# PREDICT-EPFL/polympc

Hardware: AMD Instinct MI355X
Metric: box-ADMM QP subproblem solves/s (fused SQP hot path) (higher is better)
Workload: dtype f64

## Files before the change

polympc_amd/csrc/pmpc_launch.hpp:

```cpp
#pragma once
#include <hip/hip_runtime.h>
#include <cstdlib>
#include "../../include/polympc_amd.h"
#include "pmpc_ocp.hpp"
#include "pmpc_qp.hpp"
#include "pmpc_qp_reg.hpp"
#include "pmpc_qp_reg2.hpp"
#include "pmpc_qp_cond.hpp"
#include "pmpc_qp_big.hpp"
#include "pmpc_sqp.hpp"

extern "C" pmpc_status pmpc_internal_services(pmpc_context* ctx, int P, int S, double t0, double tf, size_t ws_bytes, const void** cheb,
                                               double** ws, void** stream, size_t* lds_limit, unsigned long long** phase_cycles, int* force_lds);
extern "C" int pmpc_internal_simd_count(pmpc_context* ctx);
extern "C" int pmpc_internal_sqp_slice(pmpc_context* ctx);
extern "C" int pmpc_internal_sqp_rr(pmpc_context* ctx);
extern "C" void pmpc_internal_set_route(pmpc_context* ctx, int route);
extern "C" int pmpc_internal_last_route(pmpc_context* ctx);
enum { PMPC_SW_NO_REDO_LAUNCH = 0, PMPC_SW_NO_CONDREG = 1, PMPC_SW_NO_SCHUR = 2, PMPC_SW_SCHUR_SMALL = 3, PMPC_SW_BIG_WG4_ON = 4, PMPC_SW_BIG_WG4_OFF = 5, PMPC_SW_NO_CONDREG_RUIZ = 6 };
extern "C" int pmpc_internal_switch(pmpc_context* ctx, int which);

namespace pmpc {
using ::pmpc_status;

// ... 6 lines not shown
}

template <int NN, int MM, int NNODES> constexpr int cond_qp_staging() {
    if constexpr (NN <= WAVE) return RegKkt<NN>::TRI;
    else {
        constexpr int a = RegKkt2<NN, PMPC_COND_NV>::TRI, b = CondDims<NN, MM>::TAB_OFF + CondDims<NN, MM>::template tab_doubles<NNODES>();
        return a > b ? a : b;
    }
}

template <int NN, int MM, int NNODES, int NX> constexpr int cond_qp_staging_ws() {
    constexpr int a = cond_qp_staging<NN, MM, NNODES>(), b = CondDims<NN, MM>::TAB_OFF + CondDims<NN, MM>::template tab_doubles_ws<NNODES, NX>();
    return a > b ? a : b;
}

template <class Model> __host__ __device__ inline size_t jview_doubles(int nnodes) {
    return (size_t)nnodes * (Model::NX + Model::NG) * OcpDims<Model>::JBS;
}

template <class Model> __host__ __device__ inline size_t big_scratch_doubles(int P, int S) {
    OcpDims<Model> dm(P, S);
    return ((SqpLds::doubles(dm.n, dm.m, dm.mi) + OcpLds<Model>::doubles(P, S) + QpLds::doubles_rest(dm.n, dm.m) + jview_doubles<Model>(dm.NN) + 8) + 1) & ~(size_t)1;
}

template <class Model, int NN = 0, int MM = 0, unsigned V = 0>
#ifndef PMPC_SQP_WAVES
#define PMPC_SQP_WAVES 2
#endif
#ifndef PMPC_BIG_WAVES
#define PMPC_BIG_WAVES 1
#endif
#ifndef PMPC_COND1_WAVES
#define PMPC_COND1_WAVES 1
#endif
__global__ __launch_bounds__((V & SQP_TEAM4) ? 256 : 64, ((NN > 0 && NN + MM <= 64) ? PMPC_SQP_WAVES : ((NN > 0 && (V & SQP_COND) && NN <= 64) ? PMPC_COND1_WAVES : (((V & SQP_HBM) && (V & SQP_TWO_WAVES)) ? 2 : ((V & SQP_HBM) ? PMPC_BIG_WAVES : 1))))) void sqp_kernel(Model model, const ChebData* __restrict__ cd, int B,
                                                 const double* __restrict__ x_guess, const double* __restrict__ lam_guess,
                                                 const double* __restrict__ d, const double* __restrict__ lbx,
                                                 const double* __restrict__ ubx, const double* __restrict__ lbg,
                                                 const double* __restrict__ ubg, pmpc_sqp_settings ss, pmpc_qp_settings qs,
                                                 double* __restrict__ Hws, double* __restrict__ Aws, double* __restrict__ x,
                                                 double* __restrict__ lam, pmpc_sqp_info* __restrict__ info, unsigned long long* __restrict__ phase_cycles,
                                                 double* __restrict__ Kws, int it_begin, int it_end, double* __restrict__ slice_state, unsigned lds_dyn_doubles) {
    static_assert(sqp_variant_ok<NN, V>(), "sqp_kernel: variant flags that no launcher route selects");
    constexpr bool PROF = (V & SQP_PROF) != 0, KHBM = (V & SQP_HBM) != 0, POL = (V & SQP_HOOKS) != 0, CND = (V & SQP_COND) != 0, WG4 = (V & SQP_TEAM4) != 0;
    extern __shared__ double smem[];
    const size_t lds_doubles_total = __builtin_amdgcn_groupstaticsize() / sizeof(double) + lds_dyn_doubles;
    const int b = blockIdx.x;
    if (b >= B) return;
    int flags0 = 0;
    if (it_begin == PMPC_REDO_MODE) { if (__builtin_amdgcn_readfirstlane(info[b].status) != PMPC_SQP_REDO) return; it_begin = 0; flags0 = PMPC_FLAG_ILLCOND; }
    if (it_begin != 0 && __builtin_amdgcn_readfirstlane(info[b].status) != PMPC_SQP_IN_PROGRESS) return;
    if (it_begin < 0) it_begin = __builtin_amdgcn_readfirstlane(info[b].iter);
    const int P = cd->P, S = cd->S;
    Ocp<Model> ocp(model, P, S, cd->t_scale);
    const int n = ocp.dm.n, m = ocp.dm.m, mi = ocp.dm.mi;
    QpLds qw; SqpLds v;
    double* p; double* stage0; const double* stage_end; double* big_mail = nullptr;
    if constexpr (NN == 0 && KHBM) {
        p = qw.carve_xy(smem, n, m);
        double* rhsL = p; p += n + m;
        qw.big_lds = p; p += BigKkt::LDS_DOUBLES;
        big_mail = p; p += BIG_MAIL_DOUBLES;
        ocp.Dlds = p; p += (size_t)(P + 1) * (P + 2);
        if constexpr (Model::NG == 0 && Model::NP == 0) { if (JViewRT<Model>::tab_worth_it(ocp.dm.NN)) { p += (p - smem) & 1; ocp.jtab = p; p += JViewRT<Model>::tab_doubles(ocp.dm.NN); } }
        double* Wb = Kws + (size_t)b * (BigKkt::doubles(n + m) + big_scratch_doubles<Model>(P, S));
        double* hq = Wb + BigKkt::doubles(n + m);
        hq = v.carve(hq, n, m, mi);
        stage0 = hq;
        hq = ocp.s.carve(hq, P, S);
        stage_end = hq;
        qw.carve_rest_split(hq, rhsL, n, m, Wb);
        hq += QpLds::doubles_rest(n, m);
        ocp.jblk = hq; ocp.gblk = ocp.jblk + (size_t)ocp.dm.NN * Model::NX * OcpDims<Model>::JBS; ocp.keep_blk = true;
    } else {
        p = (NN > 0) ? qw.carve_xy(smem, n, m) : qw.carve(smem, n, ss.qp_solver == 1 ? m + n : m);
        p = v.carve(p, n, m, mi);
        stage0 = p;
        p = ocp.s.carve(p, P, S);
        constexpr int QP_STAGING0 = []() constexpr {
            if constexpr (CND) return cond_qp_staging<NN, MM, NN / (Model::NX + Model::NU)>();
            else return reg_qp_staging<NN + MM>(); }();
        int QP_STAGING = QP_STAGING0;
        if constexpr (CND && POL) {
            if (ss.preconditioner == 1) QP_STAGING = cond_qp_staging_ws<NN, MM, NN / (Model::NX + Model::NU), Model::NX>();
        }
        if (NN > 0 && (size_t)(p - stage0) < (size_t)QP_STAGING + 2 + ocp.s.const_doubles(P, S)) p = stage0 + QP_STAGING + 2 + ocp.s.const_doubles(P, S);
        stage_end = p;
    }
    if constexpr (NN > 0 && (NN + MM > WAVE || CND)) {
        ocp.jblk = p; p += jview_doubles<Model>(ocp.dm.NN); ocp.gblk = ocp.jblk + (size_t)ocp.dm.NN * Model::NX * OcpDims<Model>::JBS; ocp.keep_blk = true;
    }
    double* dL = p; p += (Model::ND > 0 ? Model::ND : 1);
    const int ln = lane_id();
    ocp.d = dL;
    double* filt = nullptr;
    if constexpr (NN == 0 || POL) { filt = p; p += FILTER_LDS_DOUBLES; }
    if constexpr (WG4) {
        if (threadIdx.x >= WAVE) { big_helper_loop<Model>((BigMail<JViewRT<Model>>*)big_mail, (int)(threadIdx.x >> 6), ocp); return; }
    }
    for (int i = ln; i < Model::ND; i += WAVE) dL[i] = d[(size_t)b * Model::ND + i];
    if constexpr (NN == 0 || POL) {
        const bool carried = ss.line_search == 1 && ss.filter_state != nullptr;
        if (ln < PMPC_FILTER_STATE_DOUBLES) filt[ln] = carried ? ss.filter_state[(size_t)b * PMPC_FILTER_STATE_DOUBLES + ln] : 0.0;
    }
    double* eigw = nullptr;
    if constexpr (NN == 0 || POL) { if (ss.regularisation == 1) { eigw = p; p += 2 * (size_t)n * n; } }
    ocp.stage_constants(cd);
    if constexpr (NN == 0 && KHBM) {
        for (int i = ln; i < (P + 1) * (P + 2); i += WAVE) ocp.Dlds[i] = ocp.s.D[i];
        wsync();
        if constexpr (Model::NG == 0 && Model::NP == 0) { if (JViewRT<Model>::tab_worth_it(ocp.dm.NN)) JViewRT<Model>::build_tables(ocp.Dlds, P, ocp.dm.NN, ocp.jtab); }
    }
    double* sst = slice_state ? slice_state + (size_t)b * 2 * n : nullptr;
    constexpr bool BOUNDS_RULE = NN > 0 && (CND || NN + MM <= WAVE);
    bool loose = false;
    for (int i = ln; i < n; i += WAVE) {
        v.x[i] = (it_begin > 0) ? x[(size_t)b * n + i] : (x_guess ? x_guess[(size_t)b * n + i] : 0.0);
        const double lbi = lbx[(size_t)b * n + i], ubi = ubx[(size_t)b * n + i];
        v.lbx[i] = lbi; v.ubx[i] = ubi;
        if constexpr (BOUNDS_RULE) loose |= (i >= ocp.dm.VARX) && (lbi < -LOOSE_BOUNDS_THRESH) && (ubi > LOOSE_BOUNDS_THRESH);
        if (it_begin > 0) { v.lg[i] = sst[i]; v.step[i] = sst[n + i]; }
    }
    for (int i = ln; i < m + n; i += WAVE)
        v.lam[i] = (it_begin > 0) ? lam[(size_t)b * (m + n) + i] : (lam_guess ? lam_guess[(size_t)b * (m + n) + i] : 0.0);
    for (int i = ln; i < mi; i += WAVE) {
        v.lbg[i] = lbg ? lbg[(size_t)b * mi + i] : -INFINITY;
        v.ubg[i] = ubg ? ubg[(size_t)b * mi + i] : INFINITY;
    }
    wsync();
    if constexpr (BOUNDS_RULE) {
        if (it_begin == 0 && flags0 == 0 && __builtin_amdgcn_ballot_w64(loose) != 0) {
            for (int i = ln; i < n; i += WAVE) x[(size_t)b * n + i] = v.x[i];
            for (int i = ln; i < m + n; i += WAVE) lam[(size_t)b * (m + n) + i] = v.lam[i];
            if (ln == 0) { pmpc_sqp_info r; r.iter = 0; r.qp_solver_iter = 0; r.status = PMPC_SQP_REDO; r.flags = PMPC_FLAG_ILLCOND; r.primal_norm = 0.0; r.dual_norm = 0.0; r.max_violation = 0.0; r.cost = 0.0; info[b] = r; }
            return;
        }
    }
    double* K0 = Hws + (size_t)b * (size_t)(n + m) * n;
    (void)Aws;
    SqpDevice<Model, NN, MM, V> sqp(ocp, v, qw, K0, K0 + n, ss, qs);
    sqp.big_mail = big_mail;
    sqp.filt = filt;
    sqp.eig = eigw;
    sqp.trace = ss.iteration_trace ? ss.iteration_trace + (size_t)b * (size_t)ss.iteration_trace_capacity * PMPC_TRACE_DOUBLES : nullptr;
    sqp.tr = ocp.s.fval;
    if constexpr (NN + MM > 112) sqp.tr += (ocp.s.fval - smem) & 1;
    {
        const int G = WAVE / ocp.dm.NN;
        const size_t need = (size_t)G * (m + ocp.dm.NN + 3);
        const size_t have = (size_t)(stage_end - ocp.s.fval);
        sqp.lsbuf = ocp.s.fval;
        sqp.ls_side_by_side = (G >= 2 && need <= have);
        sqp.ls_wide = sqp.ls_side_by_side && need + (size_t)2 * G * n <= have;
    }
    pmpc_sqp_info si;
    sqp.qp_flags = flags0;
    if (it_begin > 0) { const pmpc_sqp_info prev = info[b]; sqp.qp_iter_total = prev.qp_solver_iter; sqp.qp_flags = prev.flags; sqp.cost_log = prev.cost; }
    sqp.solve(si, it_begin, it_end);
    if (si.status == PMPC_SQP_IN_PROGRESS && sst) for (int i = ln; i < n; i += WAVE) { sst[i] = v.lg[i]; sst[n + i] = v.step[i]; }
    for (int i = ln; i < n; i += WAVE) x[(size_t)b * n + i] = v.x[i];
    for (int i = ln; i < m + n; i += WAVE) lam[(size_t)b * (m + n) + i] = v.lam[i];
    if (ln == 0) info[b] = si;
    if constexpr (NN == 0 || POL) {
        if (ss.line_search == 1 && ss.filter_state != nullptr && si.status != PMPC_SQP_REDO && ln < PMPC_FILTER_STATE_DOUBLES) ss.filter_state[(size_t)b * PMPC_FILTER_STATE_DOUBLES + ln] = filt[ln];
    }
    if constexpr (PROF) { if (phase_cycles && ln == 0) for (int i = 0; i < 24; ++i) atomicAdd(&phase_cycles[i], (unsigned long long)sqp.cyc[i]); }
    if constexpr (WG4) {
        if (ln == 0) ((BigMail<JViewRT<Model>>*)big_mail)->op = BIG_OP_EXIT;
        __syncthreads();
    }
}
template <class Model, int PP, int SS> constexpr int schur_lds_doubles_ct() {
    using SD = SchurDims<Model, PP, SS>;
    return SD::LDS_DOUBLES + SD::NNODES * SD::DD  + (SD::NPAR ? 2 * SD::N : 0)  + SD::NNODES * SD::NX * SD::JBS ;
}
template <class Model, int PP, int SS> inline size_t sqp_schur_lds_bytes(bool pol = false) {
    using SD = SchurDims<Model, PP, SS>;
    OcpDims<Model> dm(PP, SS);
    size_t stage = OcpLds<Model>::doubles(PP, SS);
    const size_t need = (size_t)RegKkt<SD::M>::TRI + OcpLds<Model>::const_doubles(PP, SS) + 8;
    if (stage < need) stage = need;
    return ((size_t)(2 * dm.n + dm.m) + SqpLds::doubles(dm.n, dm.m, dm.mi) + stage + schur_lds_doubles_ct<Model, PP, SS>() + (Model::ND > 0 ? Model::ND : 1) + (pol ? FILTER_LDS_DOUBLES : 0) + 2) * sizeof(double);
}
template <class Model, int PP, int SS, unsigned V = 0>
__global__ __launch_bounds__(64, (SchurDims<Model, PP, SS>::N + SchurDims<Model, PP, SS>::M <= 64) ? PMPC_SQP_WAVES : 1)
void sqp_schur_kernel(Model model, const ChebData* __restrict__ cd, int B, const double* __restrict__ x_guess, const double* __restrict__ lam_guess,
                      const double* __restrict__ d, const double* __restrict__ lbx, const double* __restrict__ ubx, pmpc_sqp_settings ss,
                      pmpc_qp_settings qs, double* __restrict__ x, double* __restrict__ lam, pmpc_sqp_info* __restrict__ info,
                      unsigned long long* __restrict__ phase_cycles) {
    static_assert((V & ~(SQP_PROF | SQP_HOOKS)) == 0, "sqp_schur_kernel: phase timers and the line-search hook are its only variants");
    constexpr bool PROF = (V & SQP_PROF) != 0, POL = (V & SQP_HOOKS) != 0;
    using SD = SchurDims<Model, PP, SS>;
    extern __shared__ double smem[];
    const int b = blockIdx.x;
    if (b >= B) return;
    Ocp<Model> ocp(model, PP, SS, cd->t_scale);
    constexpr int n = SD::N, m = SD::M;
    QpLds qw; SqpLds v;
    double* p = qw.carve_xy(smem, n, m);
    p = v.carve(p, n, m, 0);
    double* stage0 = p;
    p = ocp.s.carve(p, PP, SS);
    if ((size_t)(p - stage0) < (size_t)RegKkt<m>::TRI + 2 + ocp.s.const_doubles(PP, SS)) p = stage0 + RegKkt<m>::TRI + 2 + ocp.s.const_doubles(PP, SS);
    const double* stage_end = p;
    ocp.jblk = p; p += SD::NNODES * SD::NX * SD::JBS; ocp.gblk = ocp.jblk; ocp.keep_blk = true;
    double* hblk = p; p += SD::NNODES * SD::DD;
    double* hbrd = p; p += (SD::NPAR ? 2 * SD::N : 0);
    double* qblk = p; p += SD::NNODES * SD::DD;
    double* xsc = p; p += n + 1;
    double* dsc = p; p += m + 1;
    p += ((p - smem) & 1);
    double* dtab = p; p += SD::TAB;
    double* dL = p; p += (Model::ND > 0 ? Model::ND : 1);
    double* filt = nullptr;
// ... 48 lines not shown
    double *Hws, *Aws; hipStream_t stream; size_t lds_limit;
    unsigned long long* phase;
    double* slice_state; int slice_iters;
};
template <class Kernel> inline bool set_lds_attr(Kernel kern, size_t lds) {
    return hipFuncSetAttribute((const void*)kern, hipFuncAttributeMaxDynamicSharedMemorySize, (int)lds) == hipSuccess;
}
inline pmpc_status launch_status() { return (hipGetLastError() == hipSuccess) ? PMPC_OK : PMPC_ERR_HIP; }

constexpr int RR_QUEUES = 8;
constexpr int RR_LINE = 32;
constexpr int RR_HEADER_WORDS = RR_QUEUES * 3 * RR_LINE;
constexpr int RR_PASS_SHIFT = 24;
constexpr int RR_MAX_BATCH = (1 << RR_PASS_SHIFT) - 2;
constexpr int RR_MAX_ITER = 127;
constexpr int RR_SPIN_LIMIT = 1 << 16;
#ifndef PMPC_RR_HARD_TENTHS
#define PMPC_RR_HARD_TENTHS 14
#endif
constexpr int RR_HARD_TENTHS = PMPC_RR_HARD_TENTHS;
inline size_t rr_queue_bytes(int B, int max_iter) { return ((size_t)RR_HEADER_WORDS + (size_t)B * (size_t)(max_iter > 0 ? max_iter : 1)) * sizeof(int); }
__host__ __device__ inline int rr_queue_len(int B, int q) { return (q < B) ? (B - q + RR_QUEUES - 1) / RR_QUEUES : 0; }

template <class Model>
__global__ __launch_bounds__(256) void sqp_rr_init_kernel(int* __restrict__ queue, pmpc_sqp_info* __restrict__ info, int B, int max_iter) {
    const int i = blockIdx.x * blockDim.x + threadIdx.x;
    if (i < B) { pmpc_sqp_info z; z.iter = 0; z.qp_solver_iter = 0; z.status = PMPC_SQP_IN_PROGRESS; z.flags = 0; z.primal_norm = 0.0; z.dual_norm = 0.0; z.max_violation = 0.0; z.cost = 0.0; info[i] = z; }
    if (i < RR_HEADER_WORDS) {
        const int q = i / (3 * RR_LINE), w = i - q * 3 * RR_LINE;
        queue[i] = (w == RR_LINE) ? rr_queue_len(B, q) : 0;
    }
    if (i < B * max_iter) {
        int start = 0, val = 0;
        for (int q = 0; q < RR_QUEUES; ++q) {
            const int nk = rr_queue_len(B, q), cap = nk * max_iter;
            if (i >= start && i < start + cap) { const int k = i - start; val = (k < nk) ? (q + RR_QUEUES * k + 1) : 0; }
            start += cap;
        }
        queue[RR_HEADER_WORDS + i] = val;
    }
}

template <class Model, int NN, int MM, unsigned V>
__global__ __launch_bounds__(64, PMPC_SQP_WAVES) void sqp_kernel_rr(Model model, const ChebData* __restrict__ cd, int B,
                                                 const double* __restrict__ x_guess, const double* __restrict__ lam_guess,
                                                 const double* __restrict__ d, const double* __restrict__ lbx,
                                                 const double* __restrict__ ubx, const double* __restrict__ lbg,
                                                 const double* __restrict__ ubg, pmpc_sqp_settings ss, pmpc_qp_settings qs,
                                                 double* __restrict__ Hws, double* __restrict__ x, double* __restrict__ lam, pmpc_sqp_info* __restrict__ info,
                                                 double* __restrict__ slice_state, int* __restrict__ queue, unsigned lds_dyn_doubles, unsigned long long* __restrict__ prof) {
    static_assert(NN > 0 && NN + MM <= WAVE && (V & ~SQP_BLOCK_BFGS) == 0, "round-robin execution exists for the one-row-per-lane register path, default hooks");
    extern __shared__ double smem[];
    const int P = cd->P, S = cd->S;
    Ocp<Model> ocp(model, P, S, cd->t_scale);
    const int n = ocp.dm.n, m = ocp.dm.m, mi = ocp.dm.mi;
    QpLds qw; SqpLds v;
    double* p = qw.carve_xy(smem, n, m);
    p = v.carve(p, n, m, mi);
    double* stage0 = p;
    p = ocp.s.carve(p, P, S);
    if ((size_t)(p - stage0) < (size_t)reg_qp_staging<NN + MM>() + 2 + ocp.s.const_doubles(P, S)) p = stage0 + reg_qp_staging<NN + MM>() + 2 + ocp.s.const_doubles(P, S);
    const double* stage_end = p;
    double* dL = p; p += (Model::ND > 0 ? Model::ND : 1);
    ocp.d = dL;
    const int ln = lane_id();
    ocp.stage_constants(cd);
    unsigned xcc;
    asm volatile("s_getreg_b32 %0, hwreg(HW_REG_XCC_ID, 0, 4)" : "=s"(xcc));
    xcc &= (unsigned)(RR_QUEUES - 1);
    const int nk = rr_queue_len(B, (int)xcc);
    if (nk == 0) return;
    const int cap = nk * ss.max_iter;
    int start = 0;
    for (int q = 0; q < (int)xcc; ++q) start += rr_queue_len(B, q) * ss.max_iter;
    int* head = queue + (size_t)xcc * 3 * RR_LINE;
    int* tail = head + RR_LINE;
    int* finished = head + 2 * RR_LINE;
    int* entries = queue + RR_HEADER_WORDS + start;
    const int G = WAVE / ocp.dm.NN;
    const bool side_by_side = (G >= 2 && (size_t)G * (m + ocp.dm.NN + 3) <= (size_t)(stage_end - ocp.s.fval));
#ifdef PMPC_RR_PROFILE
    long long pc[5] = {0, 0, 0, 0, 0}; int items = 0; const long long life0 = clock64();
#define RR_EXIT do { if (prof && ln == 0) { atomicAdd(&prof[0], (unsigned long long)(clock64() - life0)); for (int i_ = 1; i_ < 5; ++i_) atomicAdd(&prof[i_], (unsigned long long)pc[i_]); atomicAdd(&prof[5], (unsigned long long)items); atomicAdd(&prof[6], 1ull); } return; } while (0)
#define RR_T(var) const long long var = clock64()
#define RR_ACC(i, a, b) pc[i] += (b) - (a)
#else
#define RR_EXIT return
#define RR_T(var)
#define RR_ACC(i, a, b)
    (void)prof;
#endif
    long long cyc_sum = 0; int cyc_items = 0;
    while (true) {
        RR_T(t0);
        int hq = 0;
        if (ln == 0) hq = __hip_atomic_fetch_add(head, 1, __ATOMIC_RELAXED, __HIP_MEMORY_SCOPE_AGENT);
        hq = __builtin_amdgcn_readfirstlane(hq);
        if (hq >= cap) RR_EXIT;
        int e = __builtin_amdgcn_readfirstlane(__hip_atomic_load(&entries[hq], __ATOMIC_RELAXED, __HIP_MEMORY_SCOPE_AGENT));
        for (int spin = 0; e == 0; ++spin) {
            if (spin >= RR_SPIN_LIMIT) RR_EXIT;
            if (__builtin_amdgcn_readfirstlane(__hip_atomic_load(finished, __ATOMIC_RELAXED, __HIP_MEMORY_SCOPE_AGENT)) >= nk) RR_EXIT;
            __builtin_amdgcn_s_sleep(8);
            e = __builtin_amdgcn_readfirstlane(__hip_atomic_load(&entries[hq], __ATOMIC_RELAXED, __HIP_MEMORY_SCOPE_AGENT));
        }
        const int b = (e & ((1 << RR_PASS_SHIFT) - 1)) - 1;
        const int pass = (int)((unsigned)e >> RR_PASS_SHIFT);
        RR_T(t1);
        __builtin_amdgcn_fence(__ATOMIC_ACQUIRE, "agent");
        for (int i = ln; i < Model::ND; i += WAVE) dL[i] = d[(size_t)b * Model::ND + i];
        double* sst = slice_state + (size_t)b * 2 * n;
        bool loose = false;
        for (int i = ln; i < n; i += WAVE) {
            v.x[i] = (pass > 0) ? x[(size_t)b * n + i] : (x_guess ? x_guess[(size_t)b * n + i] : 0.0);
            const double lbi = lbx[(size_t)b * n + i], ubi = ubx[(size_t)b * n + i];
            v.lbx[i] = lbi; v.ubx[i] = ubi;
// ... 424 lines not shown
```

polympc_amd/csrc/pmpc_ocp.hpp:

```cpp
#pragma once
#include <hip/hip_runtime.h>
#include "pmpc_ad.hpp"
#include "pmpc_models.hpp"
#include "pmpc_qp.hpp"

namespace pmpc {

constexpr int MAX_P = 15;
constexpr int MAX_NODES = 64;

struct ChebData {
    int P, S, NN, _pad;
    double t_start, t_stop, t_scale;
    double D[(MAX_P + 1) * (MAX_P + 1)];
    double w[MAX_P + 1];
    double tn[MAX_NODES];
};

template <class Model>
struct OcpDims {
    enum { NX = Model::NX, NU = Model::NU, NP = Model::NP, ND = Model::ND, NG = Model::NG, NDER = NX + NU + NP,
           JBS = NDER | 1 };
    int NN, VARX, VARU, n, me, mi, m;
    __host__ __device__ OcpDims(int P, int S) {
        NN = P * S + 1; VARX = NX * NN; VARU = NU * NN; n = VARX + VARU + NP; me = VARX; mi = NG * NN; m = me + mi;
    }
    __host__ __device__ int gidx(int k, int i) const {
        return i < NX ? k * NX + i : (i < NX + NU ? VARX + k * NU + (i - NX) : VARX + VARU + (i - NX - NU));
    }
};

template <class Model>
struct OcpLds {
    using Dm = OcpDims<Model>;
    enum { NX = Dm::NX, NU = Dm::NU, NP = Dm::NP, NG = Dm::NG, NDER = Dm::NDER };
    double *D, *w, *tn;
    double *nd, *nw1, *nw2; int* nsr;
    double *fval, *fjac, *Lval, *Lgrad, *gval, *gjac;
    double *Lhes, *dhes;
    double *Mval, *Mgrad, *Mhes;
    double *DX;
    __host__ __device__ static size_t doubles(int P, int S) {
        const int NN = P * S + 1;
        return const_doubles(P, S) + (size_t)NN * (NX + NX * NDER + 1 + NDER + NG + NG * NDER + 2 * NDER * NDER + NX) +
               1 + NDER + NDER * NDER + 8;
    }
    __host__ __device__ static size_t const_doubles(int P, int S) {
        const int NN = P * S + 1;
        return (size_t)(P + 1) * (P + 1) + (P + 1)  + (P + 1) + NN + 3 * (size_t)NN + (size_t)(NN + 1) / 2;
    }
    __device__ __forceinline__ double* carve(double* p, int P, int S) {
        const int NN = P * S + 1;
        D = p; p += (P + 1) * (P + 1) + (P + 1); w = p; p += P + 1; tn = p; p += NN;
        nd = p; p += NN; nw1 = p; p += NN; nw2 = p; p += NN; nsr = (int*)p; p += (NN + 1) / 2;
        fval = p; p += NN * NX; fjac = p; p += NN * NX * NDER; Lval = p; p += NN; Lgrad = p; p += NN * NDER;
        gval = p; p += NN * NG; gjac = p; p += NN * NG * NDER; Lhes = p; p += NN * NDER * NDER; dhes = p; p += NN * NDER * NDER;
        Mval = p; p += 1; Mgrad = p; p += NDER; Mhes = p; p += NDER * NDER; DX = p; p += NN * NX;
        return p;
    }
};

template <class Model>
struct Ocp {
    using Dm = OcpDims<Model>;
    enum { NX = Dm::NX, NU = Dm::NU, NP = Dm::NP, ND = Dm::ND, NG = Dm::NG, NDER = Dm::NDER };
    using ad1 = Dual<double, NDER>;
    using ad2c = Dual<ad1, 1>;

    const Model& model;
    Dm dm;
    int P, S;
    double ts;
    OcpLds<Model> s;
    const double* d;
    double* jblk = nullptr; double* gblk = nullptr; bool keep_blk = false;
    double* jtab = nullptr;
    double* Dlds = nullptr;

    __device__ Ocp(const Model& mdl, int P_, int S_, double t_scale) : model(mdl), dm(P_, S_), P(P_), S(S_), ts(t_scale), d(nullptr) {}

    __device__ __forceinline__ void stage_constants(const ChebData* cd) {
        const int ln = lane_id();
        for (int i = ln; i < (P + 1) * (P + 1); i += WAVE) s.D[i] = cd->D[i];
        for (int i = ln; i <= P; i += WAVE) s.D[(P + 1) * (P + 1) + i] = -cd->D[(P - i) * (P + 1)];
        for (int i = ln; i <= P; i += WAVE) s.w[i] = cd->w[i];
        for (int i = ln; i < dm.NN; i += WAVE) s.tn[i] = cd->tn[i];
        for (int k = ln; k < dm.NN; k += WAVE) {
            int seg, row;
            if (k == dm.NN - 1) { seg = S - 1; row = P; } else { seg = k / P; row = k % P; }
            const bool closes = (k % P == 0) && k > 0, inside = k < dm.NN - 1;
            s.nsr[k] = (closes ? (1 << 30) : 0) | (inside ? (1 << 29) : 0) | (seg << 5) | row;
            s.nd[k] = inside ? cd->D[row + row * (P + 1)] * 1.0 : -cd->D[0];
            s.nw1[k] = ts * cd->w[P];
            s.nw2[k] = ts * cd->w[k % P];
        }
        wsync();
    }

    __device__ __forceinline__ void seg_row(int k, int& seg, int& row) const {
        const int v = s.nsr[k];
        seg = (v >> 5) & 0xffffff; row = v & 31;
    }

    __device__ __forceinline__ void constraints(const double* var, double* c) {
        for (int k = lane_id(); k < dm.NN; k += WAVE) {
            double f[NX > 0 ? NX : 1];
            for (int q = 0; q < NX; ++q) f[q] = 0.0;
            const Value tk(s.tn[k]);
            model.template dynamics_impl<Value>(as_cvalues(var + k * NX), as_cvalues(var + dm.VARX + k * NU),
                                                as_cvalues(var + dm.VARX + dm.VARU), cref<double>(d), tk, as_values(f));
            int seg, row; seg_row(k, seg, row);
            for (int q = 0; q < NX; ++q) {
                double acc = 0.0;
                for (int j = 0; j <= P; ++j) acc += s.D[row + j * (P + 1)] * var[(seg * P + j) * NX + q];
                double cv = acc;
                cv -= ts * f[q];
                c[k * NX + q] = cv;
            }
            if (NG > 0) {
                double g[NG > 0 ? NG : 1];
                for (int q = 0; q < NG; ++q) g[q] = 0.0;
                model.template inequality_constraints_impl<Value>(as_cvalues(var + k * NX), as_cvalues(var + dm.VARX + k * NU),
                                                                  as_cvalues(var + dm.VARX + dm.VARU), cref<double>(d), tk.v, as_values(g));
                for (int q = 0; q < NG; ++q) c[dm.me + k * NG + q] = g[q];
            }
        }
        wsync();
    }

    __device__ __forceinline__ double cost(const double* var) {
        for (int k = lane_id(); k < dm.NN; k += WAVE) {
            Value L(0.0);
            model.template lagrange_term_impl<Value>(as_cvalues(var + k * NX), as_cvalues(var + dm.VARX + k * NU),
                                                     as_cvalues(var + dm.VARX + dm.VARU), cref<double>(d), s.tn[k], L);
            s.Lval[k] = L.v;
        }
        wsync();
        double c = 0.0;
        for (int sg = 0; sg < S; ++sg)
            for (int k = 0; k <= P; ++k) c += ts * s.w[k] * s.Lval[sg * P + k];
// ... 325 lines not shown
```

polympc_amd/csrc/pmpc_qp.hpp:

```cpp
#pragma once
#include <hip/hip_runtime.h>
#include <type_traits>
#include "../../include/polympc_amd.h"

namespace pmpc {

constexpr int WAVE = 64;
#ifndef PMPC_BIG_MEM_BATCH
#define PMPC_BIG_MEM_BATCH 32
#endif
constexpr int BIG_MEM_BATCH = PMPC_BIG_MEM_BATCH;
constexpr double RHO_MIN = 1e-6, RHO_MAX = 1e+6, RHO_EQ_FACTOR = 1e+3;
constexpr double LOOSE_BOUNDS_THRESH = 1e+10, EQ_TOL = 1e-4;
constexpr double DIV_BY_ZERO_REGUL = 10e-10;
constexpr double PMPC_SCHUR_COND_GATE = 1e7;
constexpr double PMPC_COND_GATE = 1e10;

__device__ __forceinline__ int lane_id() { int l = threadIdx.x & (WAVE - 1); asm volatile("" : "+v"(l)); return l; }
__device__ __forceinline__ void wfence() { __builtin_amdgcn_fence(__ATOMIC_SEQ_CST, "wavefront"); }
__device__ __forceinline__ void wsync() { wfence(); __builtin_amdgcn_wave_barrier(); }

__device__ __forceinline__ unsigned opaque_zero() { unsigned z = 0; asm volatile("" : "+v"(z)); return z; }

template <int CTRL, int ROW_MASK>
__device__ __forceinline__ double dpp_max_step(double v) {
    const int lo = __builtin_amdgcn_update_dpp(__double2loint(v), __double2loint(v), CTRL, ROW_MASK, 0xf, false);
    const int hi = __builtin_amdgcn_update_dpp(__double2hiint(v), __double2hiint(v), CTRL, ROW_MASK, 0xf, false);
    return fmax(v, __hiloint2double(hi, lo));
}
__device__ __forceinline__ double wave_max(double v) {
    v = dpp_max_step<0xB1, 0xf>(v);
    v = dpp_max_step<0x4E, 0xf>(v);
    v = dpp_max_step<0x141, 0xf>(v);
    v = dpp_max_step<0x140, 0xf>(v);
    v = dpp_max_step<0x142, 0xa>(v);
    v = dpp_max_step<0x143, 0xc>(v);
    const int lo = __builtin_amdgcn_readlane(__double2loint(v), 63);
    const int hi = __builtin_amdgcn_readlane(__double2hiint(v), 63);
    return __hiloint2double(hi, lo);
}
__device__ __forceinline__ void swap32(double& a, double& b) {
    const auto lo = __builtin_amdgcn_permlane32_swap(__double2loint(a), __double2loint(b), false, false);
    const auto hi = __builtin_amdgcn_permlane32_swap(__double2hiint(a), __double2hiint(b), false, false);
    a = __hiloint2double(hi[0], lo[0]); b = __hiloint2double(hi[1], lo[1]);
}
__device__ __forceinline__ void swap16(double& a, double& b) {
    const auto lo = __builtin_amdgcn_permlane16_swap(__double2loint(a), __double2loint(b), false, false);
    const auto hi = __builtin_amdgcn_permlane16_swap(__double2hiint(a), __double2hiint(b), false, false);
    a = __hiloint2double(hi[0], lo[0]); b = __hiloint2double(hi[1], lo[1]);
}
__device__ __forceinline__ void wave_max5(double& a, double& b, double& c, double& d, double& e, unsigned lane) {
    double e2 = e;
    swap32(a, b); swap32(c, d); swap32(e, e2);
    double p = fmax(a, b), q = fmax(c, d), t = fmax(e, e2);
    double t2 = t;
    swap16(p, q); swap16(t, t2);
    const double s = fmax(p, q); t = fmax(t, t2);
    const bool up = (lane & 8u) != 0;
    const double keep = up ? t : s, give = up ? s : t;
    const int glo = __builtin_amdgcn_update_dpp(__double2loint(give), __double2loint(give), 0x128, 0xf, 0xf, false);
    const int ghi = __builtin_amdgcn_update_dpp(__double2hiint(give), __double2hiint(give), 0x128, 0xf, 0xf, false);
    double u = fmax(keep, __hiloint2double(ghi, glo));
    u = dpp_max_step<0xB1, 0xf>(u);
    u = dpp_max_step<0x4E, 0xf>(u);
    u = dpp_max_step<0x141, 0xf>(u);
    auto from = [&](int l) { return __hiloint2double(__builtin_amdgcn_readlane(__double2hiint(u), l), __builtin_amdgcn_readlane(__double2loint(u), l)); };
    a = from(0); c = from(16); b = from(32); d = from(48); e = from(8);
}
template <int CTRL, int ROW_MASK>
__device__ __forceinline__ double dpp_add_step(double v) {
    const int lo = __builtin_amdgcn_update_dpp(0, __double2loint(v), CTRL, ROW_MASK, 0xf, false);
    const int hi = __builtin_amdgcn_update_dpp(0, __double2hiint(v), CTRL, ROW_MASK, 0xf, false);
    return v + __hiloint2double(hi, lo);
// ... 776 lines not shown
```

polympc_amd/csrc/pmpc_sqp.hpp:

```cpp
#pragma once
#include <hip/hip_runtime.h>
#include "pmpc_ocp.hpp"
#include "pmpc_qp.hpp"
#include "pmpc_jview.hpp"
#include "pmpc_qp_reg.hpp"
#include "pmpc_qp_reg2.hpp"
#include "pmpc_qp_big.hpp"
#include "pmpc_qp_schur.hpp"
#include "pmpc_qp_cond.hpp"
#include "pmpc_ruiz.hpp"
#include "pmpc_admm.hpp"

#ifndef PMPC_EXPERIMENT_FORCE_SYMLOWER
#define PMPC_EXPERIMENT_FORCE_SYMLOWER 0
#endif
#ifndef PMPC_WIDE_TERMS
#define PMPC_WIDE_TERMS 2
#endif
namespace pmpc {

template <int N_>
struct TriDeal {
    static constexpr int T = N_ * (N_ + 1) / 2, W = N_ + 1, SLOTS = (T + WAVE - 1) / WAVE;
    static constexpr unsigned MAGIC = (65536u + W - 1) / W;
    static constexpr bool magic_ok() { for (unsigned t = 0; t < (unsigned)T; ++t) if (((t * MAGIC) >> 16) != t / (unsigned)W) return false; return true; }
    static_assert(magic_ok(), "TriDeal: t / (n + 1) by multiply and shift");
    static constexpr bool slot_full(int e) { return WAVE * e + WAVE - 1 < T; }
    __device__ __forceinline__ static void entry(unsigned lane, int e, unsigned& i, unsigned& j) {
        unsigned t = lane + (unsigned)(WAVE * e);
        if (!slot_full(e)) t = t < (unsigned)T ? t : (unsigned)(T - 1);
        const unsigned R = (t * MAGIC) >> 16, c = t - R * (unsigned)W;
        const bool low = c <= R;
        i = low ? R : (unsigned)(N_ - 1) - R;
        j = low ? c : c - R - 1u;
    }
};

struct SqpLds {
    double *x, *lam, *lam_k, *h, *lg, *lgn, *al, *au, *lx, *ux, *lbx, *ubx, *lbg, *ubg, *step, *xs, *cb, *t1, *t2, *t3;
    __host__ __device__ static size_t doubles(int n, int m, int mi) {
        return 12 * (size_t)n + 2 * (size_t)(m + n) + 3 * (size_t)m + 2 * (size_t)mi + 3 * (size_t)(n + m) + 8;
    }
    __device__ __forceinline__ double* carve(double* p, int n, int m, int mi) {
        x = p; p += n; lam = p; p += m + n; lam_k = p; p += m + n; h = p; p += n; lg = p; p += n; lgn = p; p += n;
        al = p; p += m; au = p; p += m; lx = p; p += n; ux = p; p += n; lbx = p; p += n; ubx = p; p += n;
        lbg = p; p += mi; ubg = p; p += mi; step = p; p += n; xs = p; p += n; cb = p; p += m;
        t1 = p; p += n + m; t2 = p; p += n + m; t3 = p; p += n + m;
        return p;
    }
};

constexpr double DBL_EPS = 2.220446049250313e-16;
constexpr int RUIZ_MAX_NDER = 64;
constexpr int PMPC_SQP_IN_PROGRESS = 3;
constexpr int PMPC_SQP_REDO = 4;
constexpr int PMPC_REDO_MODE = -0x7fffffff - 1;

enum : unsigned { SQP_PROF = 1, SQP_BLOCK_BFGS = 2, SQP_HBM = 4, SQP_TWO_WAVES = 8, SQP_HOOKS = 16, SQP_COND = 32, SQP_TEAM4 = 64 };
template <int NN, unsigned V> constexpr bool sqp_variant_ok() {
    return (!(V & SQP_HBM) || NN == 0) &&
           (!(V & SQP_TWO_WAVES) || (V & SQP_HBM)) &&
           (!(V & SQP_TEAM4) || (V & SQP_HBM)) &&
           (!(V & SQP_COND) || NN > 0) &&
           (!(V & SQP_HOOKS) || NN > 0) &&
           (!(V & SQP_BLOCK_BFGS) || NN > 0) &&
           V < 2 * SQP_TEAM4;
}
template <class Model, int NN = 0, int MM = 0, unsigned VARIANT = 0, int PS = 0>
struct SqpDevice {
    static_assert(sqp_variant_ok<NN, VARIANT>() && PS >= 0, "SqpDevice: variant flags that no kernel is built with");
    static constexpr bool PROF = (VARIANT & SQP_PROF) != 0, BIG = (VARIANT & SQP_HBM) != 0, POL = (VARIANT & SQP_HOOKS) != 0;
    static constexpr int HU = (VARIANT & SQP_BLOCK_BFGS) ? 1 : 0;
    static constexpr bool SCH = PS > 0;
    static constexpr bool SLIM = BIG && (VARIANT & SQP_TWO_WAVES) && !(VARIANT & SQP_TEAM4);
    static constexpr int BIG_NW = (BIG && (VARIANT & SQP_TEAM4)) ? 4 : 1;
    void* big_mail = nullptr;
    static constexpr bool CND = (VARIANT & SQP_COND) != 0;
    static constexpr int SCH_P = PS / 256, SCH_S = PS % 256;
    static constexpr bool HOOKS = (NN == 0) || POL;
    using Dm = OcpDims<Model>;
    static constexpr bool RUIZ_COMPILED = HOOKS && (int)Dm::NDER <= RUIZ_MAX_NDER && PS <= 0;
    static constexpr bool REG1 = !SCH && NN > 0 && NN + MM <= WAVE;
    static constexpr bool REG2 = !SCH && NN > 0 && NN + MM > WAVE;
    double *hblk = nullptr, *hbrd = nullptr , *qblk = nullptr, *xsc = nullptr, *dsc = nullptr, *dtab = nullptr;
    static constexpr int MEMCH = BIG ? BIG_MEM_BATCH : 8;
    Ocp<Model>& ocp;
    SqpLds& v;
    QpLds& qw;
    double* lsbuf = nullptr;
    bool ls_side_by_side = false;
    bool ls_wide = false;
    bool cb_valid = false;
    double* tr = nullptr;
    double* Hw;
    double* Aw;
    int ldw;
    const pmpc_sqp_settings& ss;
    const pmpc_qp_settings& qs;
    int n, m, me, mi;
    static constexpr int NNODES_CT_ = (NN > 0) ? MM / (Model::NX + Model::NG) : 0;
    __device__ __forceinline__ int n_ct() const { if constexpr (NN > 0) return NN; else return n; }
    __device__ __forceinline__ int m_ct() const { if constexpr (NN > 0) return MM; else return m; }
    __device__ __forceinline__ int me_ct() const { if constexpr (NN > 0) return Model::NX * NNODES_CT_; else return me; }
    __device__ __forceinline__ int mi_ct() const { if constexpr (NN > 0) return Model::NG * NNODES_CT_; else return mi; }
    using JV = JView<Model, (NNODES_CT_ > 0 ? NNODES_CT_ : 1)>;
    __device__ __forceinline__ JV jview() const { return JV{ocp.s.D, ocp.s.nsr, ocp.jblk, ocp.gblk, ocp.P}; }
    double cost_log = 0.0, primal_norm = 0.0, dual_norm = 0.0, max_violation = 0.0;
    double alpha_log = 0.0; int qp_iter_last = 0, qp_status_last = 0;
    double* trace = nullptr;
    int qp_iter_total = 0;
    int qp_flags = 0;
    static constexpr int FLAG_GAVE_UP = 0x100;
    long long cyc[PROF ? 24 : 1] = {0};
    __device__ __forceinline__ static long long now() { if constexpr (PROF) return clock64(); else return 0; }
    __device__ __forceinline__ void acc(int i, long long dt) { if constexpr (PROF) cyc[i] += dt; }

#ifdef PMPC_EXPERIMENT_WG_STAMPS
    long long t_start_stamp = wall_clock64();
#endif
    __device__ SqpDevice(Ocp<Model>& o, SqpLds& v_, QpLds& q_, double* H_, double* A_, const pmpc_sqp_settings& s, const pmpc_qp_settings& q)
        : ocp(o), v(v_), qw(q_), Hw(H_), Aw(A_), ldw(o.dm.n + o.dm.m), ss(s), qs(q), n(o.dm.n), m(o.dm.m), me(o.dm.me), mi(o.dm.mi) {}

    __device__ __forceinline__ double constraints_violation(const double* xx) {
        ocp.constraints(xx, v.cb);
        double cl1 = DBL_EPS;
        double s = 0.0;
        for (int i = 0; i < me; ++i) s += fabs(v.cb[i]);
        cl1 += s;
        s = 0.0; for (int i = 0; i < mi; ++i) s += fmax(v.lbg[i] - v.cb[me + i], 0.0); cl1 += s;
        s = 0.0; for (int i = 0; i < mi; ++i) s += fmax(v.cb[me + i] - v.ubg[i], 0.0); cl1 += s;
        s = 0.0; for (int i = 0; i < n; ++i) s += fmax(v.lbx[i] - xx[i], 0.0); cl1 += s;
        s = 0.0; for (int i = 0; i < n; ++i) s += fmax(xx[i] - v.ubx[i], 0.0); cl1 += s;
        wsync();
        return cl1;
    }
    __device__ __forceinline__ double max_constraints_violation(const double* xx) {
        if (!cb_valid) ocp.constraints(xx, v.cb);
        const int ln = lane_id();
        const int n = n_ct(), me = me_ct(), mi = mi_ct();
        double c = 0.0, a = -INFINITY, b = -INFINITY, e = -INFINITY, f = -INFINITY;
        for (int i = ln; i < me; i += WAVE) c = fmax(c, fabs(v.cb[i]));
        for (int i = ln; i < mi; i += WAVE) { a = fmax(a, v.lbg[i] - v.cb[me + i]); b = fmax(b, v.cb[me + i] - v.ubg[i]); }
        for (int i = ln; i < n; i += WAVE) { e = fmax(e, v.lbx[i] - xx[i]); f = fmax(f, xx[i] - v.ubx[i]); }
        c = fmax(fmax(c, fmax(a, b)), fmax(e, f));
        c = wave_max(c);
        wsync();
        return c;
    }

    double* filt = nullptr;
    __device__ __forceinline__ bool filter_mode() const { if constexpr (HOOKS) return __builtin_amdgcn_readfirstlane(ss.line_search) == 1; else return false; }
    __device__ __forceinline__ bool filter_is_acceptable(double cost, double constraint) const {
        int cnt = (int)filt[0];
        if (cnt > PMPC_FILTER_MAX_DEPTH) cnt = PMPC_FILTER_MAX_DEPTH;
        const double beta = ss.filter_beta;
        bool ok = true;
        for (int i = 0; i < cnt; ++i) {
            const double f = filt[1 + 2 * i], c = filt[2 + 2 * i];
            const double bc = beta * c;
            if (((f - bc) <= cost) && ((c - bc) <= constraint)) ok = false;
        }
        return __builtin_amdgcn_readfirstlane((int)ok) != 0;
    }
    __device__ __forceinline__ void filter_add(double cost, double constraint) {
        wsync();
        if (lane_id() == 0) {
            int cnt = (int)filt[0];
            if (cnt > PMPC_FILTER_MAX_DEPTH) cnt = PMPC_FILTER_MAX_DEPTH;
            if (cnt < ss.filter_max_depth) {
                int k = 0;
                for (int i = 0; i < cnt; ++i) {
                    const double f = filt[1 + 2 * i], c = filt[2 + 2 * i];
                    if (!((f >= cost) && (c >= constraint))) { filt[1 + 2 * k] = f; filt[2 + 2 * k] = c; ++k; }
                }
// ... 979 lines not shown
```

Before: 30.20 million.

## Use compile-time OCP dimensions and literal LDS base addresses for fixed-size kernels

```diff
diff --git a/polympc_amd/csrc/pmpc_launch.hpp b/polympc_amd/csrc/pmpc_launch.hpp
--- a/polympc_amd/csrc/pmpc_launch.hpp
+++ b/polympc_amd/csrc/pmpc_launch.hpp
@@ -82,8 +82,12 @@
     if (it_begin != 0 && __builtin_amdgcn_readfirstlane(info[b].status) != PMPC_SQP_IN_PROGRESS) return;
     if (it_begin < 0) it_begin = __builtin_amdgcn_readfirstlane(info[b].iter);
     const int P = cd->P, S = cd->S;
-    Ocp<Model> ocp(model, P, S, cd->t_scale);
+    constexpr int KN = static_nodes<Model, NN, MM>();
+    constexpr bool ROLLED = KN > 0;
+    Ocp<Model, KN> ocp(model, P, S, cd->t_scale);
     const int n = ocp.dm.n, m = ocp.dm.m, mi = ocp.dm.mi;
+    if constexpr (KN > 0) static_assert(decltype(ocp)::Dm::n == NN && decltype(ocp)::Dm::m == MM, "sqp_kernel: <NN, MM> is not a grid of this model");
+    double* const lds = lds_origin<decltype(ocp.s)::TAIL_DW>(smem);
     QpLds qw; SqpLds v;
     double* p; double* stage0; const double* stage_end; double* big_mail = nullptr;
     if constexpr (NN == 0 && KHBM) {
@@ -103,7 +107,7 @@
         hq += QpLds::doubles_rest(n, m);
         ocp.jblk = hq; ocp.gblk = ocp.jblk + (size_t)ocp.dm.NN * Model::NX * OcpDims<Model>::JBS; ocp.keep_blk = true;
     } else {
-        p = (NN > 0) ? qw.carve_xy(smem, n, m) : qw.carve(smem, n, ss.qp_solver == 1 ? m + n : m);
+        p = (NN > 0) ? qw.carve_xy(lds, n, m) : qw.carve(smem, n, ss.qp_solver == 1 ? m + n : m);
         p = v.carve(p, n, m, mi);
         stage0 = p;
         p = ocp.s.carve(p, P, S);
@@ -114,6 +118,12 @@
         if constexpr (CND && POL) {
             if (ss.preconditioner == 1) QP_STAGING = cond_qp_staging_ws<NN, MM, NN / (Model::NX + Model::NU), Model::NX>();
         }
+        if constexpr (decltype(ocp.s)::TAIL_DW) {
+            static_assert(SqpLds::carved(NN, MM, Model::NG * KN) + 2 * NN + 8 == SqpLds::doubles(NN, MM, Model::NG * KN), "SqpLds::carve ends where SqpLds::doubles says (which has always counted 2 n + 8 spare doubles)");
+            constexpr size_t NC = decltype(ocp.s)::node_const_doubles(KN), NS = decltype(ocp.s)::node_staging_doubles(KN);
+            static_assert(NC + NS + decltype(ocp.s)::dw_doubles(1) + 8 == OcpLds<Model>::doubles(1, KN - 1) && decltype(ocp.s)::dw_doubles(1) + NC == OcpLds<Model>::const_doubles(1, KN - 1), "the constant layout ends where OcpLds::doubles says");
+            if ((size_t)(p - stage0) < (size_t)QP_STAGING + 2 + NC) p = stage0 + QP_STAGING + 2 + NC;
+        } else
         if (NN > 0 && (size_t)(p - stage0) < (size_t)QP_STAGING + 2 + ocp.s.const_doubles(P, S)) p = stage0 + QP_STAGING + 2 + ocp.s.const_doubles(P, S);
         stage_end = p;
     }
@@ -125,6 +135,7 @@
     ocp.d = dL;
     double* filt = nullptr;
     if constexpr (NN == 0 || POL) { filt = p; p += FILTER_LDS_DOUBLES; }
+    if constexpr (decltype(ocp.s)::TAIL_DW) p = ocp.s.carve_dw(p, P);
     if constexpr (WG4) {
         if (threadIdx.x >= WAVE) { big_helper_loop<Model>((BigMail<JViewRT<Model>>*)big_mail, (int)(threadIdx.x >> 6), ocp); return; }
     }
@@ -144,16 +155,17 @@
     double* sst = slice_state ? slice_state + (size_t)b * 2 * n : nullptr;
     constexpr bool BOUNDS_RULE = NN > 0 && (CND || NN + MM <= WAVE);
     bool loose = false;
-    for (int i = ln; i < n; i += WAVE) {
+    const int n_rt = rolled_bound<ROLLED>(n), nm_rt = rolled_bound<ROLLED>(m + n), mi_rt = rolled_bound<ROLLED>(mi);
+    for (int i = ln; i < n_rt; i += WAVE) {
         v.x[i] = (it_begin > 0) ? x[(size_t)b * n + i] : (x_guess ? x_guess[(size_t)b * n + i] : 0.0);
         const double lbi = lbx[(size_t)b * n + i], ubi = ubx[(size_t)b * n + i];
         v.lbx[i] = lbi; v.ubx[i] = ubi;
         if constexpr (BOUNDS_RULE) loose |= (i >= ocp.dm.VARX) && (lbi < -LOOSE_BOUNDS_THRESH) && (ubi > LOOSE_BOUNDS_THRESH);
         if (it_begin > 0) { v.lg[i] = sst[i]; v.step[i] = sst[n + i]; }
     }
-    for (int i = ln; i < m + n; i += WAVE)
+    for (int i = ln; i < nm_rt; i += WAVE)
         v.lam[i] = (it_begin > 0) ? lam[(size_t)b * (m + n) + i] : (lam_guess ? lam_guess[(size_t)b * (m + n) + i] : 0.0);
-    for (int i = ln; i < mi; i += WAVE) {
+    for (int i = ln; i < mi_rt; i += WAVE) {
         v.lbg[i] = lbg ? lbg[(size_t)b * mi + i] : -INFINITY;
         v.ubg[i] = ubg ? ubg[(size_t)b * mi + i] : INFINITY;
     }
@@ -174,7 +186,7 @@
     sqp.eig = eigw;
     sqp.trace = ss.iteration_trace ? ss.iteration_trace + (size_t)b * (size_t)ss.iteration_trace_capacity * PMPC_TRACE_DOUBLES : nullptr;
     sqp.tr = ocp.s.fval;
-    if constexpr (NN + MM > 112) sqp.tr += (ocp.s.fval - smem) & 1;
+    if constexpr (NN + MM > 112) sqp.tr += (ocp.s.fval - lds) & 1;
     {
         const int G = WAVE / ocp.dm.NN;
         const size_t need = (size_t)G * (m + ocp.dm.NN + 3);
@@ -187,9 +199,10 @@
     sqp.qp_flags = flags0;
     if (it_begin > 0) { const pmpc_sqp_info prev = info[b]; sqp.qp_iter_total = prev.qp_solver_iter; sqp.qp_flags = prev.flags; sqp.cost_log = prev.cost; }
     sqp.solve(si, it_begin, it_end);
-    if (si.status == PMPC_SQP_IN_PROGRESS && sst) for (int i = ln; i < n; i += WAVE) { sst[i] = v.lg[i]; sst[n + i] = v.step[i]; }
-    for (int i = ln; i < n; i += WAVE) x[(size_t)b * n + i] = v.x[i];
-    for (int i = ln; i < m + n; i += WAVE) lam[(size_t)b * (m + n) + i] = v.lam[i];
+    const int n_out = rolled_bound<ROLLED>(n), nm_out = rolled_bound<ROLLED>(m + n);
+    if (si.status == PMPC_SQP_IN_PROGRESS && sst) for (int i = ln; i < n_out; i += WAVE) { sst[i] = v.lg[i]; sst[n + i] = v.step[i]; }
+    for (int i = ln; i < n_out; i += WAVE) x[(size_t)b * n + i] = v.x[i];
+    for (int i = ln; i < nm_out; i += WAVE) lam[(size_t)b * (m + n) + i] = v.lam[i];
     if (ln == 0) info[b] = si;
     if constexpr (NN == 0 || POL) {
         if (ss.line_search == 1 && ss.filter_state != nullptr && si.status != PMPC_SQP_REDO && ln < PMPC_FILTER_STATE_DOUBLES) ss.filter_state[(size_t)b * PMPC_FILTER_STATE_DOUBLES + ln] = filt[ln];
@@ -344,16 +357,19 @@
     static_assert(NN > 0 && NN + MM <= WAVE && (V & ~SQP_BLOCK_BFGS) == 0, "round-robin execution exists for the one-row-per-lane register path, default hooks");
     extern __shared__ double smem[];
     const int P = cd->P, S = cd->S;
-    Ocp<Model> ocp(model, P, S, cd->t_scale);
+    constexpr int KN = static_nodes<Model, NN, MM>();
+    Ocp<Model, KN> ocp(model, P, S, cd->t_scale);
     const int n = ocp.dm.n, m = ocp.dm.m, mi = ocp.dm.mi;
     QpLds qw; SqpLds v;
-    double* p = qw.carve_xy(smem, n, m);
+    double* p = qw.carve_xy(lds_origin<decltype(ocp.s)::TAIL_DW>(smem), n, m);
     p = v.carve(p, n, m, mi);
     double* stage0 = p;
     p = ocp.s.carve(p, P, S);
-    if ((size_t)(p - stage0) < (size_t)reg_qp_staging<NN + MM>() + 2 + ocp.s.const_doubles(P, S)) p = stage0 + reg_qp_staging<NN + MM>() + 2 + ocp.s.const_doubles(P, S);
+    const size_t cst_ahead = decltype(ocp.s)::TAIL_DW ? decltype(ocp.s)::node_const_doubles(KN) : ocp.s.const_doubles(P, S);
+    if ((size_t)(p - stage0) < (size_t)reg_qp_staging<NN + MM>() + 2 + cst_ahead) p = stage0 + reg_qp_staging<NN + MM>() + 2 + cst_ahead;
     const double* stage_end = p;
     double* dL = p; p += (Model::ND > 0 ? Model::ND : 1);
+    if constexpr (decltype(ocp.s)::TAIL_DW) p = ocp.s.carve_dw(p, P);
     ocp.d = dL;
     const int ln = lane_id();
     ocp.stage_constants(cd);
diff --git a/polympc_amd/csrc/pmpc_ocp.hpp b/polympc_amd/csrc/pmpc_ocp.hpp
--- a/polympc_amd/csrc/pmpc_ocp.hpp
+++ b/polympc_amd/csrc/pmpc_ocp.hpp
@@ -17,6 +17,10 @@
     double tn[MAX_NODES];
 };
 
+#ifndef PMPC_STATIC_LAYOUT
+#define PMPC_STATIC_LAYOUT 2
+#endif
+
 template <class Model>
 struct OcpDims {
     enum { NX = Model::NX, NU = Model::NU, NP = Model::NP, ND = Model::ND, NG = Model::NG, NDER = NX + NU + NP,
@@ -30,9 +34,28 @@
     }
 };
 
-template <class Model>
+template <class Model, int KN>
+struct OcpDimsCT {
+    static_assert(KN > 0, "OcpDimsCT: a compile-time node count");
+    enum { NX = Model::NX, NU = Model::NU, NP = Model::NP, ND = Model::ND, NG = Model::NG, NDER = NX + NU + NP, JBS = OcpDims<Model>::JBS };
+    static constexpr int NN = KN, VARX = NX * KN, VARU = NU * KN, n = VARX + VARU + NP, me = VARX, mi = NG * KN, m = me + mi;
+    __host__ __device__ OcpDimsCT(int, int) {}
+    __host__ __device__ static constexpr int gidx(int k, int i) {
+        return i < NX ? k * NX + i : (i < NX + NU ? VARX + k * NU + (i - NX) : VARX + VARU + (i - NX - NU));
+    }
+};
+template <class Model, int KN> struct OcpDimsSel { using type = OcpDimsCT<Model, KN>; };
+template <class Model> struct OcpDimsSel<Model, 0> { using type = OcpDims<Model>; };
+template <class Model, int NN, int MM> constexpr int static_nodes() { return (PMPC_STATIC_LAYOUT >= 1 && NN > 0) ? MM / (Model::NX + Model::NG) : 0; }
+template <bool OPAQUE> __device__ __forceinline__ int rolled_bound(int v) {
+    if constexpr (OPAQUE) asm volatile("" : "+s"(v));
+    return v;
+}
+
+template <class Model, int KN = 0>
 struct OcpLds {
-    using Dm = OcpDims<Model>;
+    using Dm = typename OcpDimsSel<Model, KN>::type;
+    static constexpr bool TAIL_DW = KN > 0 && PMPC_STATIC_LAYOUT >= 2;
     enum { NX = Dm::NX, NU = Dm::NU, NP = Dm::NP, NG = Dm::NG, NDER = Dm::NDER };
     double *D, *w, *tn;
     double *nd, *nw1, *nw2; int* nsr;
@@ -40,18 +63,25 @@
     double *Lhes, *dhes;
     double *Mval, *Mgrad, *Mhes;
     double *DX;
-    __host__ __device__ static size_t doubles(int P, int S) {
+    __host__ __device__ static constexpr size_t doubles(int P, int S) {
         const int NN = P * S + 1;
         return const_doubles(P, S) + (size_t)NN * (NX + NX * NDER + 1 + NDER + NG + NG * NDER + 2 * NDER * NDER + NX) +
                1 + NDER + NDER * NDER + 8;
     }
-    __host__ __device__ static size_t const_doubles(int P, int S) {
+    __host__ __device__ static constexpr size_t const_doubles(int P, int S) {
         const int NN = P * S + 1;
         return (size_t)(P + 1) * (P + 1) + (P + 1)  + (P + 1) + NN + 3 * (size_t)NN + (size_t)(NN + 1) / 2;
     }
+    __host__ __device__ static constexpr size_t dw_doubles(int P) { return (size_t)(P + 1) * (P + 1) + (P + 1)  + (P + 1); }
+    __host__ __device__ static constexpr size_t node_const_doubles(int NN) { return (size_t)NN + 3 * (size_t)NN + (size_t)(NN + 1) / 2; }
+    __host__ __device__ static constexpr size_t node_staging_doubles(int NN) {
+        return (size_t)NN * (NX + NX * NDER + 1 + NDER + NG + NG * NDER + 2 * NDER * NDER + NX) + 1 + NDER + NDER * NDER;
+    }
+    __device__ __forceinline__ double* carve_dw(double* p, int P) { D = p; p += (P + 1) * (P + 1) + (P + 1); w = p; p += P + 1; return p; }
     __device__ __forceinline__ double* carve(double* p, int P, int S) {
-        const int NN = P * S + 1;
-        D = p; p += (P + 1) * (P + 1) + (P + 1); w = p; p += P + 1; tn = p; p += NN;
+        const int NN = KN > 0 ? KN : P * S + 1;
+        if constexpr (!TAIL_DW) p = carve_dw(p, P);
+        tn = p; p += NN;
         nd = p; p += NN; nw1 = p; p += NN; nw2 = p; p += NN; nsr = (int*)p; p += (NN + 1) / 2;
         fval = p; p += NN * NX; fjac = p; p += NN * NX * NDER; Lval = p; p += NN; Lgrad = p; p += NN * NDER;
         gval = p; p += NN * NG; gjac = p; p += NN * NG * NDER; Lhes = p; p += NN * NDER * NDER; dhes = p; p += NN * NDER * NDER;
@@ -60,9 +90,10 @@
     }
 };
 
-template <class Model>
+template <class Model, int KN = 0>
 struct Ocp {
-    using Dm = OcpDims<Model>;
+    using Dm = typename OcpDimsSel<Model, KN>::type;
+    static constexpr bool STATIC = KN > 0;
     enum { NX = Dm::NX, NU = Dm::NU, NP = Dm::NP, ND = Dm::ND, NG = Dm::NG, NDER = Dm::NDER };
     using ad1 = Dual<double, NDER>;
     using ad2c = Dual<ad1, 1>;
@@ -71,7 +102,7 @@
     Dm dm;
     int P, S;
     double ts;
-    OcpLds<Model> s;
+    OcpLds<Model, KN> s;
     const double* d;
     double* jblk = nullptr; double* gblk = nullptr; bool keep_blk = false;
     double* jtab = nullptr;
@@ -84,8 +115,9 @@
         for (int i = ln; i < (P + 1) * (P + 1); i += WAVE) s.D[i] = cd->D[i];
         for (int i = ln; i <= P; i += WAVE) s.D[(P + 1) * (P + 1) + i] = -cd->D[(P - i) * (P + 1)];
         for (int i = ln; i <= P; i += WAVE) s.w[i] = cd->w[i];
-        for (int i = ln; i < dm.NN; i += WAVE) s.tn[i] = cd->tn[i];
-        for (int k = ln; k < dm.NN; k += WAVE) {
+        const int nn_rt = rolled_bound<STATIC>(dm.NN);
+        for (int i = ln; i < nn_rt; i += WAVE) s.tn[i] = cd->tn[i];
+        for (int k = ln; k < nn_rt; k += WAVE) {
             int seg, row;
             if (k == dm.NN - 1) { seg = S - 1; row = P; } else { seg = k / P; row = k % P; }
             const bool closes = (k % P == 0) && k > 0, inside = k < dm.NN - 1;
diff --git a/polympc_amd/csrc/pmpc_qp.hpp b/polympc_amd/csrc/pmpc_qp.hpp
--- a/polympc_amd/csrc/pmpc_qp.hpp
+++ b/polympc_amd/csrc/pmpc_qp.hpp
@@ -19,6 +19,11 @@
 __device__ __forceinline__ int lane_id() { int l = threadIdx.x & (WAVE - 1); asm volatile("" : "+v"(l)); return l; }
 __device__ __forceinline__ void wfence() { __builtin_amdgcn_fence(__ATOMIC_SEQ_CST, "wavefront"); }
 __device__ __forceinline__ void wsync() { wfence(); __builtin_amdgcn_wave_barrier(); }
+
+template <bool LITERAL> __device__ __forceinline__ double* lds_origin(double* smem) {
+    if constexpr (LITERAL) { typedef __attribute__((address_space(3))) double lds_double; return (double*)(lds_double*)(size_t)sizeof(double) - 1; }
+    else return smem;
+}
 
 __device__ __forceinline__ unsigned opaque_zero() { unsigned z = 0; asm volatile("" : "+v"(z)); return z; }
 
diff --git a/polympc_amd/csrc/pmpc_sqp.hpp b/polympc_amd/csrc/pmpc_sqp.hpp
--- a/polympc_amd/csrc/pmpc_sqp.hpp
+++ b/polympc_amd/csrc/pmpc_sqp.hpp
@@ -38,8 +38,11 @@
 
 struct SqpLds {
     double *x, *lam, *lam_k, *h, *lg, *lgn, *al, *au, *lx, *ux, *lbx, *ubx, *lbg, *ubg, *step, *xs, *cb, *t1, *t2, *t3;
-    __host__ __device__ static size_t doubles(int n, int m, int mi) {
+    __host__ __device__ static constexpr size_t doubles(int n, int m, int mi) {
         return 12 * (size_t)n + 2 * (size_t)(m + n) + 3 * (size_t)m + 2 * (size_t)mi + 3 * (size_t)(n + m) + 8;
+    }
+    __host__ __device__ static constexpr size_t carved(int n, int m, int mi) {
+        return (size_t)n + (m + n) + (m + n) + n + n + n + m + m + n + n + n + n + mi + mi + n + n + m + (n + m) + (n + m) + (n + m);
     }
     __device__ __forceinline__ double* carve(double* p, int n, int m, int mi) {
         x = p; p += n; lam = p; p += m + n; lam_k = p; p += m + n; h = p; p += n; lg = p; p += n; lgn = p; p += n;
@@ -78,13 +81,15 @@
     static constexpr bool CND = (VARIANT & SQP_COND) != 0;
     static constexpr int SCH_P = PS / 256, SCH_S = PS % 256;
     static constexpr bool HOOKS = (NN == 0) || POL;
-    using Dm = OcpDims<Model>;
+    static constexpr int OCP_KN = (PS > 0) ? 0 : static_nodes<Model, NN, MM>();
+    using OcpT = Ocp<Model, OCP_KN>;
+    using Dm = typename OcpT::Dm;
     static constexpr bool RUIZ_COMPILED = HOOKS && (int)Dm::NDER <= RUIZ_MAX_NDER && PS <= 0;
     static constexpr bool REG1 = !SCH && NN > 0 && NN + MM <= WAVE;
     static constexpr bool REG2 = !SCH && NN > 0 && NN + MM > WAVE;
     double *hblk = nullptr, *hbrd = nullptr , *qblk = nullptr, *xsc = nullptr, *dsc = nullptr, *dtab = nullptr;
     static constexpr int MEMCH = BIG ? BIG_MEM_BATCH : 8;
-    Ocp<Model>& ocp;
+    OcpT& ocp;
     SqpLds& v;
     QpLds& qw;
     double* lsbuf = nullptr;
@@ -118,8 +123,9 @@
 #ifdef PMPC_EXPERIMENT_WG_STAMPS
     long long t_start_stamp = wall_clock64();
 #endif
-    __device__ SqpDevice(Ocp<Model>& o, SqpLds& v_, QpLds& q_, double* H_, double* A_, const pmpc_sqp_settings& s, const pmpc_qp_settings& q)
-        : ocp(o), v(v_), qw(q_), Hw(H_), Aw(A_), ldw(o.dm.n + o.dm.m), ss(s), qs(q), n(o.dm.n), m(o.dm.m), me(o.dm.me), mi(o.dm.mi) {}
+    __device__ SqpDevice(OcpT& o, SqpLds& v_, QpLds& q_, double* H_, double* A_, const pmpc_sqp_settings& s, const pmpc_qp_settings& q)
+        : ocp(o), v(v_), qw(q_), Hw(H_), Aw(A_), ldw(o.dm.n + o.dm.m), ss(s), qs(q), n(rolled_bound<(OCP_KN > 0)>(o.dm.n)), m(rolled_bound<(OCP_KN > 0)>(o.dm.m)),
+          me(rolled_bound<(OCP_KN > 0)>(o.dm.me)), mi(rolled_bound<(OCP_KN > 0)>(o.dm.mi)) {}
 
     __device__ __forceinline__ double constraints_violation(const double* xx) {
         ocp.constraints(xx, v.cb);
```

Result: faster. 31.40 million, median of 6 (+4.0%).
